# xiexh20/VisTracker

Measured on AMD Instinct MI355X. Metric: frames/sec joint SMPL+object fit, higher is better.
Workload: dtype f32 (decoder GEMMs: 22-bit split-f16 operands x3 MFMA, fp32 accumulate)

## Files before the change

vistracker_amd/csrc/smplh.hip:

```cpp
#include "common.h"
#include <cstring>

#define V_ VT_SMPL_V
#define J_ VT_SMPL_J
#define NB_ VT_SMPL_NB
#define NP_ VT_SMPL_NP
#define VP_ 6912
#define NVT_ 27
#define KQ_ 472
#define NQ_ 480
typedef float f32x4 __attribute__((ext_vector_type(4)));
#define MFMA16(a, b, c) __builtin_amdgcn_mfma_f32_16x16x4f32((a), (b), (c), 0, 0, 0)

#define WS_R 0
#define WS_J (52 * 9)
#define WS_G (WS_J + 52 * 3)
#define WS_A (WS_G + 52 * 12)
#define WS_FRAME (WS_A + 52 * 12)
#define PT_DA 0
#define PT_DTR 624
#define PT_N 627
#define KTOT_ (VP_ * 3)
#define KG_SLAB 24
#define NKS_ (KTOT_ / 16 / KG_SLAB)

#define SCHED_STEPS 32
#define SCHED_WIDTH 10
struct SmplParents { int p[J_]; int nsteps; short sched[SCHED_STEPS][SCHED_WIDTH]; };

#define SP_K 8
struct vt_smplh {
    float *Q_kcv, *Q_t, *W_jv, *W_v64, *J_t, *J_s;
    float *W_sp;
    int nnz;
    SmplParents par;
};

struct RodCtx { float n, ax, ay, az, c, s, qn, w, x, y, z; };

__device__ __forceinline__ void rodrigues_fwd(const float *t, float *R, RodCtx *k)
{
    const float xe = t[0] + 1e-8f, ye = t[1] + 1e-8f, ze = t[2] + 1e-8f;
    const float n = sqrtf(xe * xe + ye * ye + ze * ze);
    const float ax = t[0] / n, ay = t[1] / n, az = t[2] / n;
    const float h = n * 0.5f;
    const float c = cosf(h), s = sinf(h);
    const float q0 = c, q1 = s * ax, q2 = s * ay, q3 = s * az;
    const float qn = sqrtf(q0 * q0 + q1 * q1 + q2 * q2 + q3 * q3);
    const float w = q0 / qn, x = q1 / qn, y = q2 / qn, z = q3 / qn;
    const float w2 = w * w, x2 = x * x, y2 = y * y, z2 = z * z;
    const float wx = w * x, wy = w * y, wz = w * z, xy = x * y, xz = x * z, yz = y * z;
    R[0] = w2 + x2 - y2 - z2; R[1] = 2 * xy - 2 * wz;   R[2] = 2 * wy + 2 * xz;
    R[3] = 2 * wz + 2 * xy;   R[4] = w2 - x2 + y2 - z2; R[5] = 2 * yz - 2 * wx;
    R[6] = 2 * xz - 2 * wy;   R[7] = 2 * wx + 2 * yz;   R[8] = w2 - x2 - y2 + z2;
    if (k) { k->n = n; k->ax = ax; k->ay = ay; k->az = az; k->c = c; k->s = s; k->qn = qn; k->w = w; k->x = x; k->y = y; k->z = z; }
}

__device__ __forceinline__ void rodrigues_bwd(const float *t, const float *dR, float *dt)
{
    float R[9]; RodCtx k; rodrigues_fwd(t, R, &k);
    const float w = k.w, x = k.x, y = k.y, z = k.z;
    const float dw = 2 * w * (dR[0] + dR[4] + dR[8]) + 2 * (-z * dR[1] + y * dR[2] + z * dR[3] - x * dR[5] - y * dR[6] + x * dR[7]);
    const float dx = 2 * x * (dR[0] - dR[4] - dR[8]) + 2 * (y * dR[1] + z * dR[2] + y * dR[3] - w * dR[5] + z * dR[6] + w * dR[7]);
    const float dy = 2 * y * (-dR[0] + dR[4] - dR[8]) + 2 * (x * dR[1] + w * dR[2] + x * dR[3] + z * dR[5] - w * dR[6] + z * dR[7]);
    const float dz = 2 * z * (-dR[0] - dR[4] + dR[8]) + 2 * (-w * dR[1] + x * dR[2] + w * dR[3] + y * dR[5] + x * dR[6] + y * dR[7]);
    const float dot = w * dw + x * dx + y * dy + z * dz;
    const float dq0 = (dw - w * dot) / k.qn, dq1 = (dx - x * dot) / k.qn, dq2 = (dy - y * dot) / k.qn, dq3 = (dz - z * dot) / k.qn;
    const float dh = -k.s * dq0 + k.c * (k.ax * dq1 + k.ay * dq2 + k.az * dq3);
    const float dax = k.s * dq1, day = k.s * dq2, daz = k.s * dq3;
    const float dn = 0.5f * dh - (t[0] * dax + t[1] * day + t[2] * daz) / (k.n * k.n);
    dt[0] = dax / k.n + dn * (t[0] + 1e-8f) / k.n;
    dt[1] = day / k.n + dn * (t[1] + 1e-8f) / k.n;
    dt[2] = daz / k.n + dn * (t[2] + 1e-8f) / k.n;
}

__global__ void rodrigues_fwd_kernel(const float *aa, int n, float *R)
{
    const int i = blockIdx.x * blockDim.x + threadIdx.x;
    if (i >= n) return;
    float t[3] = {aa[3 * i], aa[3 * i + 1], aa[3 * i + 2]}, r[9];
    rodrigues_fwd(t, r, nullptr);
#pragma unroll
    for (int e = 0; e < 9; e++) R[9 * i + e] = r[e];
}

__global__ void rodrigues_bwd_kernel(const float *aa, int n, const float *dR, float *daa)
{
    const int i = blockIdx.x * blockDim.x + threadIdx.x;
    if (i >= n) return;
    float t[3] = {aa[3 * i], aa[3 * i + 1], aa[3 * i + 2]}, g[9], d[3];
#pragma unroll
    for (int e = 0; e < 9; e++) g[e] = dR[9 * i + e];
    rodrigues_bwd(t, g, d);
    daa[3 * i] = d[0]; daa[3 * i + 1] = d[1]; daa[3 * i + 2] = d[2];
}

__global__ __launch_bounds__(64) void smplh_pose_kernel(const float *__restrict__ pose, const float *__restrict__ betas,
                                                        const float *__restrict__ trans, const float *__restrict__ J_t,
                                                        const float *__restrict__ J_s, SmplParents par,
                                                        float *__restrict__ ws, float *__restrict__ jtr, const int *skip)
{
    VT_SKIP_RETURN(skip);
    __shared__ float sR[J_ * 9], sJ[J_ * 3], sG[J_ * 12];
    const int b = blockIdx.x, j = threadIdx.x;
    float *w = ws + (size_t)b * WS_FRAME;
    if (j < J_) {
        float t[3] = {pose[(b * J_ + j) * 3], pose[(b * J_ + j) * 3 + 1], pose[(b * J_ + j) * 3 + 2]}, R[9];
        rodrigues_fwd(t, R, nullptr);
#pragma unroll
        for (int e = 0; e < 9; e++) { sR[j * 9 + e] = R[e]; w[WS_R + j * 9 + e] = R[e]; }
#pragma unroll
        for (int c = 0; c < 3; c++) {
            float a = J_t[j * 3 + c];
#pragma unroll
            for (int l = 0; l < NB_; l++) a += J_s[(j * 3 + c) * NB_ + l] * betas[b * NB_ + l];
            sJ[j * 3 + c] = a; w[WS_J + j * 3 + c] = a;
        }
    }
    __shared__ int sPar[J_];
    if (j < J_) sPar[j] = par.p[j];
    __syncthreads();
    int lvl = 0, maxl = 0;
    if (j < J_) { for (int q = j; q != 0; q = sPar[q]) lvl++; }
    maxl = lvl;
    for (int o = 32; o > 0; o >>= 1) maxl = max(maxl, __shfl_xor(maxl, o, 64));
    maxl = __builtin_amdgcn_readfirstlane(maxl);
    if (j == 0) { for (int r = 0; r < 3; r++) { for (int c = 0; c < 3; c++) sG[r * 4 + c] = sR[r * 3 + c]; sG[r * 4 + 3] = sJ[r]; } }
    __syncthreads();
    for (int l = 1; l <= maxl; l++) {
        if (j < J_ && lvl == l) {
            const int i = j, p = sPar[i];
            const float *Gp = sG + 12 * p, *Ri = sR + 9 * i;
            const float d0 = sJ[3 * i] - sJ[3 * p], d1 = sJ[3 * i + 1] - sJ[3 * p + 1], d2 = sJ[3 * i + 2] - sJ[3 * p + 2];
            float *Gi = sG + 12 * i;
            for (int r = 0; r < 3; r++) {
                const float g0 = Gp[r * 4], g1 = Gp[r * 4 + 1], g2 = Gp[r * 4 + 2];
                Gi[r * 4 + 0] = g0 * Ri[0] + g1 * Ri[3] + g2 * Ri[6];
                Gi[r * 4 + 1] = g0 * Ri[1] + g1 * Ri[4] + g2 * Ri[7];
                Gi[r * 4 + 2] = g0 * Ri[2] + g1 * Ri[5] + g2 * Ri[8];
                Gi[r * 4 + 3] = g0 * d0 + g1 * d1 + g2 * d2 + Gp[r * 4 + 3];
            }
        }
        __syncthreads();
    }
    if (j < J_) {
        const float *G = sG + 12 * j;
#pragma unroll
        for (int r = 0; r < 3; r++) {
            const float gt = G[r * 4 + 3];
            w[WS_G + j * 12 + r * 4 + 0] = G[r * 4]; w[WS_G + j * 12 + r * 4 + 1] = G[r * 4 + 1];
            w[WS_G + j * 12 + r * 4 + 2] = G[r * 4 + 2]; w[WS_G + j * 12 + r * 4 + 3] = gt;
            w[WS_A + j * 12 + r * 4 + 0] = G[r * 4]; w[WS_A + j * 12 + r * 4 + 1] = G[r * 4 + 1]; w[WS_A + j * 12 + r * 4 + 2] = G[r * 4 + 2];
            w[WS_A + j * 12 + r * 4 + 3] = gt - (G[r * 4] * sJ[3 * j] + G[r * 4 + 1] * sJ[3 * j + 1] + G[r * 4 + 2] * sJ[3 * j + 2]);
            if (jtr) jtr[(b * J_ + j) * 3 + r] = gt + trans[3 * b + r];
        }
    }
}

#define FWD_FB 16
#ifndef FWD_PF
#define FWD_PF 6
#endif
#define AXS 516
#define SAS 628
#define FWD_R0 (FWD_FB * AXS > 8 * SAS ? FWD_FB * AXS : 8 * SAS)
__global__ __launch_bounds__(256) void smplh_verts_kernel(const float *__restrict__ Q_kcv, const float *__restrict__ W_jv,
                                                          const float *__restrict__ betas, const float *__restrict__ trans,
                                                          const float *__restrict__ ws, int B,
                                                          float *__restrict__ verts, float *__restrict__ v_posed, const float *__restrict__ W_sp, int nnz, const int *skip)
{
    VT_SKIP_RETURN(skip);
    extern __shared__ __attribute__((aligned(16))) float lds[];
    float *sAx = lds;
    float *sA = lds;
    float *sVp = lds + FWD_R0;
    float *sW = sVp + FWD_FB * 64 * 3;
    float *sTr = sW + (nnz > 0 ? 2 * SP_K * 64 : J_ * 64);
    const int tid = threadIdx.x, wave = tid >> 6, lane = tid & 63, q = lane >> 4, j = lane & 15;
    const int b0 = blockIdx.y * FWD_FB, v = blockIdx.x * 64 + wave * 16 + j;
    for (int k = tid; k < KQ_; k += 256) {
        const int e9 = k % 9;
        const float sub = (k < NP_ && (e9 == 0 || e9 == 4 || e9 == 8)) ? 1.f : 0.f;
        float val[FWD_FB];
#pragma unroll
        for (int f = 0; f < FWD_FB; f++) {
            const int b = min(b0 + f, B - 1);
            if (k < NP_) val[f] = ws[(size_t)b * WS_FRAME + WS_R + 9 + k];
            else if (k < NP_ + NB_) val[f] = betas[b * NB_ + (k - NP_)];
            else val[f] = (k == NP_ + NB_) ? 1.f : 0.f;
        }
#pragma unroll
        for (int f = 0; f < FWD_FB; f++) sAx[f * AXS + k] = val[f] - sub;
    }
    if (nnz > 0) {
        for (int i = tid; i < nnz * 64; i += 256) {
            sW[i] = W_sp[(size_t)(i >> 6) * VP_ + blockIdx.x * 64 + (i & 63)];
            sW[SP_K * 64 + i] = W_sp[(size_t)(SP_K + (i >> 6)) * VP_ + blockIdx.x * 64 + (i & 63)];
        }
    } else
        for (int i = tid; i < J_ * 64; i += 256) sW[i] = W_jv[(i >> 6) * VP_ + blockIdx.x * 64 + (i & 63)];
    if (tid < FWD_FB * 3) { const int f = tid / 3, b = min(b0 + f, B - 1); sTr[tid] = trans[b * 3 + tid % 3]; }
    __syncthreads();

    f32x4 acc[3];
#pragma unroll
    for (int c = 0; c < 3; c++) acc[c] = (f32x4){0.f, 0.f, 0.f, 0.f};
    constexpr int NS = KQ_ / 8;
    float bq[FWD_PF][2][3];
#define FWD_LOADQ(slot_, s_)                                                                     \
    {                                                                                            \
        const float *qk = Q_kcv + (size_t)(8 * (s_) + 2 * q) * 3 * VP_ + v;                      \
        _Pragma("unroll") for (int e = 0; e < 2; e++)                                            \
            _Pragma("unroll") for (int c = 0; c < 3; c++) bq[slot_][e][c] = qk[(size_t)(e * 3 + c) * VP_]; \
    }
#pragma unroll
    for (int s = 0; s < FWD_PF; s++) FWD_LOADQ(s, s)
#pragma unroll
    for (int s = 0; s < NS; s++) {
        const float2 av = *reinterpret_cast<const float2 *>(sAx + j * AXS + 8 * s + 2 * q);
#pragma unroll
        for (int c = 0; c < 3; c++) acc[c] = MFMA16(av.x, bq[s % FWD_PF][0][c], acc[c]);
#pragma unroll
        for (int c = 0; c < 3; c++) acc[c] = MFMA16(av.y, bq[s % FWD_PF][1][c], acc[c]);
        if (s + FWD_PF < NS) FWD_LOADQ(s % FWD_PF, s + FWD_PF)
        __builtin_amdgcn_sched_barrier(0);
    }
#undef FWD_LOADQ
    __syncthreads();
#pragma unroll
    for (int r = 0; r < 4; r++)
#pragma unroll
        for (int c = 0; c < 3; c++) sVp[((4 * q + r) * 64 + wave * 16 + j) * 3 + c] = acc[c][r];
    const int vv = tid & 63, vg = blockIdx.x * 64 + vv;
#pragma unroll 1
    for (int r = 0; r < 4; r++) {
        if ((r & 1) == 0) {
            if (r) __syncthreads();
            for (int i = tid; i < 8 * 624; i += 256) {
                const int sl = i / 624, f = 4 * (sl >> 1) + r + (sl & 1), b = min(b0 + f, B - 1);
                sA[sl * SAS + (i % 624)] = ws[(size_t)b * WS_FRAME + WS_A + (i % 624)];
            }
            __syncthreads();
        }
        const int f = 4 * wave + r, b = b0 + f;
        float T[12];
#pragma unroll
        for (int e = 0; e < 12; e++) T[e] = 0.f;
        const float4 *Af = reinterpret_cast<const float4 *>(sA + (2 * wave + (r & 1)) * SAS);
        if (nnz > 0) {
            for (int k = 0; k < nnz; k++) {
                const int jj = __float_as_int(sW[k * 64 + vv]);
                const float wj = sW[(SP_K + k) * 64 + vv];
                const float4 a0 = Af[jj * 3], a1 = Af[jj * 3 + 1], a2 = Af[jj * 3 + 2];
                T[0] += wj * a0.x; T[1] += wj * a0.y; T[2] += wj * a0.z; T[3] += wj * a0.w;
                T[4] += wj * a1.x; T[5] += wj * a1.y; T[6] += wj * a1.z; T[7] += wj * a1.w;
                T[8] += wj * a2.x; T[9] += wj * a2.y; T[10] += wj * a2.z; T[11] += wj * a2.w;
            }
        } else {
#pragma unroll 4
            for (int jj = 0; jj < J_; jj++) {
                const float wj = sW[jj * 64 + vv];
                const float4 a0 = Af[jj * 3], a1 = Af[jj * 3 + 1], a2 = Af[jj * 3 + 2];
                T[0] += wj * a0.x; T[1] += wj * a0.y; T[2] += wj * a0.z; T[3] += wj * a0.w;
                T[4] += wj * a1.x; T[5] += wj * a1.y; T[6] += wj * a1.z; T[7] += wj * a1.w;
                T[8] += wj * a2.x; T[9] += wj * a2.y; T[10] += wj * a2.z; T[11] += wj * a2.w;
            }
        }
        if (b < B && vg < V_) {
            const float p0 = sVp[(f * 64 + vv) * 3], p1 = sVp[(f * 64 + vv) * 3 + 1], p2 = sVp[(f * 64 + vv) * 3 + 2];
            const size_t o = ((size_t)b * V_ + vg) * 3;
#pragma unroll
            for (int rr = 0; rr < 3; rr++) verts[o + rr] = T[rr * 4] * p0 + T[rr * 4 + 1] * p1 + T[rr * 4 + 2] * p2 + T[rr * 4 + 3] + sTr[f * 3 + rr];
            v_posed[o] = p0; v_posed[o + 1] = p1; v_posed[o + 2] = p2;
        }
    }
}

template <int FB>
__global__ __launch_bounds__(256) void smplh_bwd_tile_kernel(const float *__restrict__ W_v64, const float *__restrict__ ws,
                                                             const float *__restrict__ v_posed, const float *__restrict__ dverts,
                                                             int B, float *__restrict__ part, float *__restrict__ dvp_g, const int *skip)
{
    VT_SKIP_RETURN(skip);
    extern __shared__ __attribute__((aligned(16))) float lds[];
    float *sdT = lds;
    float *sA = sdT + 256 * 13;
    const int tid = threadIdx.x, tile = blockIdx.x, b0 = blockIdx.y * FB, v0 = tile * 256, v = v0 + tid;
    const int wave = tid >> 6, lane = tid & 63, q = lane >> 4, j = lane & 15;
    for (int i = tid; i < FB * 624; i += 256) { const int f = i / 624, b = min(b0 + f, B - 1); sA[i] = ws[(size_t)b * WS_FRAME + WS_A + (i % 624)]; }
    float w1[4][13], w2[64];
#pragma unroll
    for (int mt = 0; mt < 4; mt++)
#pragma unroll
        for (int ks = 0; ks < 13; ks++) w1[mt][ks] = W_v64[(size_t)(v0 + 64 * wave + 16 * mt + j) * 64 + 4 * ks + q];
#pragma unroll
    for (int ks = 0; ks < 64; ks++) w2[ks] = W_v64[(size_t)(v0 + 4 * ks + q) * 64 + wave * 16 + j];
    __syncthreads();
    float dvn[3] = {0.f, 0.f, 0.f}, vpn[3] = {0.f, 0.f, 0.f};
    auto fetch = [&](int b) {
#pragma unroll
        for (int r = 0; r < 3; r++) { dvn[r] = 0.f; vpn[r] = 0.f; }
        if (b < B && v < V_) {
            const size_t o = ((size_t)b * V_ + v) * 3;
            dvn[0] = dverts[o]; dvn[1] = dverts[o + 1]; dvn[2] = dverts[o + 2];
            vpn[0] = v_posed[o]; vpn[1] = v_posed[o + 1]; vpn[2] = v_posed[o + 2];
        }
    };
    fetch(b0);
#pragma unroll 1
    for (int f = 0; f < FB; f++) {
        const int b = b0 + f;
        const float dv[3] = {dvn[0], dvn[1], dvn[2]}, vp[3] = {vpn[0], vpn[1], vpn[2]};
        if (f + 1 < FB) fetch(b + 1);
#pragma unroll
        for (int r = 0; r < 3; r++) {
            sdT[tid * 13 + r * 4 + 0] = dv[r] * vp[0]; sdT[tid * 13 + r * 4 + 1] = dv[r] * vp[1];
            sdT[tid * 13 + r * 4 + 2] = dv[r] * vp[2]; sdT[tid * 13 + r * 4 + 3] = dv[r];
        }
        __syncthreads();
        {
            f32x4 t[4];
#pragma unroll
            for (int mt = 0; mt < 4; mt++) t[mt] = (f32x4){0.f, 0.f, 0.f, 0.f};
#pragma unroll
            for (int ks = 0; ks < 13; ks++) {
                const float bv = j < 12 ? sA[f * 624 + (4 * ks + q) * 12 + j] : 0.f;
#pragma unroll
                for (int mt = 0; mt < 4; mt++) t[mt] = MFMA16(w1[mt][ks], bv, t[mt]);
            }
            const int r4 = (j < 12 ? (j >> 2) : 0) * 4 + 3;
#pragma unroll
            for (int mt = 0; mt < 4; mt++) {
#pragma unroll
                for (int r = 0; r < 4; r++) {
                    const int vl = 64 * wave + 16 * mt + 4 * q + r;
                    float x = t[mt][r] * sdT[vl * 13 + r4];
                    x += __shfl_down(x, 4, 16) + __shfl_down(x, 8, 16);
                    if (j < 3 && b < B) dvp_g[(size_t)b * KTOT_ + (size_t)(v0 + vl) * 3 + j] = x;
                }
            }
        }
        {
            f32x4 acc = (f32x4){0.f, 0.f, 0.f, 0.f}, acc2 = (f32x4){0.f, 0.f, 0.f, 0.f};
#pragma unroll
            for (int ks = 0; ks < 64; ks += 2) {
                const int va = 4 * ks + q, vb = va + 4;
                const float a0 = j < 12 ? sdT[va * 13 + j] : 0.f, a1 = j < 12 ? sdT[vb * 13 + j] : 0.f;
                acc = MFMA16(a0, w2[ks], acc);
                acc2 = MFMA16(a1, w2[ks + 1], acc2);
            }
            acc += acc2;
            if (b < B) {
                float *dst = part + ((size_t)tile * B + b) * PT_N;
                const int jn = wave * 16 + j;
#pragma unroll
                for (int r = 0; r < 4; r++) {
                    const int e = 4 * q + r;
                    if (e < 12) {
                        if (jn < J_) dst[PT_DA + jn * 12 + e] = acc[r];
                        else if (jn == J_ && (e & 3) == 3) dst[PT_DTR + (e >> 2)] = acc[r];
                    }
                }
            }
        }
        __syncthreads();
    }
}

#define BL_M 96
#ifndef BL_NW
#define BL_NW 1
#endif
#define BL_AS 132
__global__ __launch_bounds__(256) void smplh_bwd_blend_kernel(const float *__restrict__ Q_p, const float *__restrict__ dvp_g, int B,
                                                              float *__restrict__ part3, const int *skip)
{
    VT_SKIP_RETURN(skip);
    __shared__ __attribute__((aligned(16))) float sA[BL_M * BL_AS];
    const int tid = threadIdx.x, wave = tid >> 6, lane = tid & 63, q = lane >> 4, j = lane & 15;
    const int ks = blockIdx.x, m0 = blockIdx.z * BL_M, nt0 = blockIdx.y * (4 * BL_NW) + wave * BL_NW;
    f32x4 acc[6][BL_NW];
#pragma unroll
    for (int mt = 0; mt < 6; mt++)
#pragma unroll
        for (int n = 0; n < BL_NW; n++) acc[mt][n] = (f32x4){0.f, 0.f, 0.f, 0.f};
    const float4 *Q4 = reinterpret_cast<const float4 *>(Q_p);
#pragma unroll 1
    for (int c = 0; c < KG_SLAB / 8; c++) {
        __syncthreads();
        for (int i = tid; i < BL_M * 32; i += 256) {
            const int row = i >> 5, c4 = i & 31, b = m0 + row;
            float4 v = make_float4(0.f, 0.f, 0.f, 0.f);
            if (b < B) v = *reinterpret_cast<const float4 *>(dvp_g + (size_t)b * KTOT_ + (size_t)(ks * KG_SLAB + c * 8) * 16 + c4 * 4);
            *reinterpret_cast<float4 *>(sA + row * BL_AS + c4 * 4) = v;
        }
        __syncthreads();
#pragma unroll
        for (int g = 0; g < 8; g++) {
            const size_t kg = (size_t)ks * KG_SLAB + c * 8 + g;
            float bq[BL_NW][4];
#pragma unroll
            for (int n = 0; n < BL_NW; n++) {
                const float4 fq = Q4[(kg * (NQ_ / 16) + min(nt0 + n, NQ_ / 16 - 1)) * 64 + lane];
                bq[n][0] = fq.x; bq[n][1] = fq.y; bq[n][2] = fq.z; bq[n][3] = fq.w;
            }
#pragma unroll
            for (int mt = 0; mt < 6; mt++) {
                const float4 a4 = *reinterpret_cast<const float4 *>(sA + (mt * 16 + j) * BL_AS + g * 16 + q * 4);
                const float av[4] = {a4.x, a4.y, a4.z, a4.w};
#pragma unroll
                for (int s = 0; s < 4; s++)
#pragma unroll
                    for (int n = 0; n < BL_NW; n++) acc[mt][n] = MFMA16(av[s], bq[n][s], acc[mt][n]);
            }
        }
    }
#pragma unroll
    for (int mt = 0; mt < 6; mt++) {
#pragma unroll
        for (int r = 0; r < 4; r++) {
            const int b = m0 + mt * 16 + 4 * q + r;
            if (b < B) {
                float *dst = part3 + ((size_t)ks * B + b) * NQ_;
#pragma unroll
                for (int n = 0; n < BL_NW; n++)
                    if (nt0 + n < NQ_ / 16) dst[(nt0 + n) * 16 + j] = acc[mt][n][r];
            }
        }
    }
}

__global__ __launch_bounds__(256) void smplh_bwd_frame_kernel(const float *__restrict__ pose, const float *__restrict__ J_s,
                                                              SmplParents par, const float *__restrict__ ws,
                                                              const float *__restrict__ part, const float *__restrict__ part3,
                                                              const float *__restrict__ djtr, int B, float *__restrict__ dpose, float *__restrict__ dbetas,
                                                              float *__restrict__ dtrans, const int *skip)
{
    VT_SKIP_RETURN(skip);
    __shared__ float red[PT_N], red3[NQ_];
    __shared__ float sdG[J_ * 12], sdJ[J_ * 3], sdR[J_ * 9];
    __shared__ float sG[J_ * 12], sRm[J_ * 9], sJr[J_ * 3];
    const int b = blockIdx.x, tid = threadIdx.x;
    const float *w = ws + (size_t)b * WS_FRAME;
    for (int i = tid; i < J_ * 12; i += 256) sG[i] = w[WS_G + i];
    for (int i = tid; i < J_ * 9; i += 256) sRm[i] = w[WS_R + i];
    for (int i = tid; i < J_ * 3; i += 256) sJr[i] = w[WS_J + i];
    for (int i = tid; i < PT_N; i += 256) {
        float s = 0.f;
#pragma unroll 9
        for (int t = 0; t < NVT_; t++) s += part[((size_t)t * B + b) * PT_N + i];
        red[i] = s;
    }
    for (int i = tid; i < NQ_; i += 256) {
        float s = 0.f;
#pragma unroll 9
        for (int t = 0; t < NKS_; t++) s += part3[((size_t)t * B + b) * NQ_ + i];
        red3[i] = s;
    }
    __syncthreads();
    if (tid < J_) {
        const int j = tid;
        const float *G = sG + 12 * j; const float *Jr = sJr;
        float dj[3] = {0.f, 0.f, 0.f};
#pragma unroll
        for (int r = 0; r < 3; r++) {
            const float dat = red[PT_DA + 12 * j + r * 4 + 3];
#pragma unroll
            for (int c = 0; c < 3; c++) { sdG[12 * j + r * 4 + c] = red[PT_DA + 12 * j + r * 4 + c] - dat * Jr[3 * j + c]; dj[c] -= G[r * 4 + c] * dat; }
            sdG[12 * j + r * 4 + 3] = dat + (djtr ? djtr[(b * J_ + j) * 3 + r] : 0.f);
        }
        sdJ[3 * j] = dj[0]; sdJ[3 * j + 1] = dj[1]; sdJ[3 * j + 2] = dj[2];
#pragma unroll
        for (int e = 0; e < 9; e++) sdR[9 * j + e] = 0.f;
    }
    __syncthreads();
    const int jloc = tid / 24, el = tid - 24 * jloc;
    const int nsteps = par.nsteps > 0 ? par.nsteps : J_ - 1;
    for (int step = 0; step < nsteps; step++) {
        const int j = par.nsteps > 0 ? (jloc < SCHED_WIDTH ? (int)par.sched[step][jloc < SCHED_WIDTH ? jloc : 0] : -1) : (jloc == 0 ? J_ - 1 - step : -1);
        if (j >= 1) {
            const int p = par.p[j];
            const float *Gp = sG + 12 * p, *Rj = sRm + 9 * j, *dGj = sdG + 12 * j;
            float upd = 0.f; float *dst = nullptr; float upd2 = 0.f; float *dst2 = nullptr;
            if (el < 12) {
                const int r = el >> 2, c = el & 3;
                dst = sdG + 12 * p + el;
                if (c < 3) upd = dGj[r * 4] * Rj[3 * c] + dGj[r * 4 + 1] * Rj[3 * c + 1] + dGj[r * 4 + 2] * Rj[3 * c + 2] + dGj[r * 4 + 3] * (sJr[3 * j + c] - sJr[3 * p + c]);
                else upd = dGj[r * 4 + 3];
            } else if (el < 21) {
                const int e = el - 12, r = e / 3, c = e - 3 * r;
                dst = sdR + 9 * j + e;
                upd = Gp[r] * dGj[c] + Gp[4 + r] * dGj[4 + c] + Gp[8 + r] * dGj[8 + c];
            } else {
                const int c = el - 21;
                upd = Gp[c] * dGj[3] + Gp[4 + c] * dGj[7] + Gp[8 + c] * dGj[11];
                dst = sdJ + 3 * j + c; dst2 = sdJ + 3 * p + c; upd2 = -upd;
            }
            if (dst) *dst += upd;
            if (dst2) *dst2 += upd2;
        }
        __syncthreads();
    }
    if (tid < 3) { for (int c = 0; c < 3; c++) sdR[3 * tid + c] += sdG[tid * 4 + c]; sdJ[tid] += sdG[tid * 4 + 3]; }
    __syncthreads();
    if (tid < J_) {
        const int j = tid;
        float g[9], t[3] = {pose[(b * J_ + j) * 3], pose[(b * J_ + j) * 3 + 1], pose[(b * J_ + j) * 3 + 2]}, d[3];
#pragma unroll
        for (int e = 0; e < 9; e++) g[e] = sdR[9 * j + e] + (j >= 1 ? red3[(j - 1) * 9 + e] : 0.f);
        rodrigues_bwd(t, g, d);
        dpose[(b * J_ + j) * 3] = d[0]; dpose[(b * J_ + j) * 3 + 1] = d[1]; dpose[(b * J_ + j) * 3 + 2] = d[2];
    } else if (tid >= 64 && tid < 64 + NB_) {
        const int l = tid - 64;
        float s = red3[NP_ + l];
        for (int i = 0; i < J_ * 3; i++) s += J_s[i * NB_ + l] * sdJ[i];
        dbetas[b * NB_ + l] = s;
    } else if (tid >= 128 && tid < 131) {
        const int c = tid - 128;
        float s = red[PT_DTR + c];
        if (djtr) for (int j = 0; j < J_; j++) s += djtr[(b * J_ + j) * 3 + c];
        dtrans[b * 3 + c] = s;
    }
}

extern "C" int vt_smplh_create(vt_smplh **out, const float *v_template, const float *shapedirs, const float *posedirs,
                               const float *J_regressor, const float *weights, const int *parents, void *stream)
{
    VT_REQUIRE(out && v_template && shapedirs && posedirs && J_regressor && weights && parents, "vt_smplh_create: null argument");
    hipStream_t st = vt_stream(stream);
    vt_smplh *h = new vt_smplh();
    for (int j = 0; j < J_; j++) h->par.p[j] = (j == 0) ? 0 : parents[j];
    for (int j = 1; j < J_; j++) VT_REQUIRE(h->par.p[j] >= 0 && h->par.p[j] < j, "vt_smplh_create: parents[%d]=%d must be in [0,%d)", j, parents[j], j);
    {
        int lvl[J_], rank[J_], maxl = 0;
        lvl[0] = 0; rank[0] = 0;
        for (int j = 1; j < J_; j++) { lvl[j] = lvl[h->par.p[j]] + 1; maxl = std::max(maxl, lvl[j]); rank[j] = 0; for (int k = j + 1; k < J_; k++) rank[j] += (h->par.p[k] == h->par.p[j]); }
        int n = 0; bool ok = true;
        for (int t = 0; t < SCHED_STEPS; t++) for (int i = 0; i < SCHED_WIDTH; i++) h->par.sched[t][i] = -1;
        for (int l = maxl; l >= 1 && ok; l--)
            for (int r = 0; r < J_ && ok; r++) {
                int cnt = 0;
                for (int j = J_ - 1; j >= 1; j--) if (lvl[j] == l && rank[j] == r) { if (n >= SCHED_STEPS || cnt >= SCHED_WIDTH) { ok = false; break; } h->par.sched[n][cnt++] = (short)j; }
                if (cnt) n++;
            }
        h->par.nsteps = ok ? n : 0;
    }
    float *Q_kcv = new float[(size_t)KQ_ * 3 * VP_](), *Q_t = new float[(size_t)VP_ * 3 * NQ_](), *W_jv = new float[(size_t)J_ * VP_](),
          *J_t = new float[J_ * 3], *J_s = new float[J_ * 3 * NB_];
    for (int v = 0; v < V_; v++) for (int c = 0; c < 3; c++) {
        for (int k = 0; k < NP_ + NB_ + 1; k++) {
            const float val = k < NP_ ? posedirs[((size_t)v * 3 + c) * NP_ + k]
                            : (k < NP_ + NB_ ? shapedirs[((size_t)v * 3 + c) * NB_ + (k - NP_)] : v_template[v * 3 + c]);
            Q_kcv[(size_t)(k * 3 + c) * VP_ + v] = val;
            {
                const size_t kr = (size_t)v * 3 + c, g = kr >> 4, qq = (kr & 15) >> 2, ss = kr & 3;
                Q_t[((g * (NQ_ / 16) + (k >> 4)) * 64 + qq * 16 + (k & 15)) * 4 + ss] = val;
            }
        }
    }
    float *W_v64 = new float[(size_t)VP_ * 64]();
    for (int v = 0; v < V_; v++) { for (int j = 0; j < J_; j++) { W_jv[(size_t)j * VP_ + v] = weights[(size_t)v * J_ + j]; W_v64[(size_t)v * 64 + j] = weights[(size_t)v * J_ + j]; } W_v64[(size_t)v * 64 + J_] = 1.0f; }
    float *W_sp = new float[(size_t)2 * SP_K * VP_]();
    int nnz = 0;
    for (int v = 0; v < V_; v++) {
        int k = 0;
        for (int j = 0; j < J_; j++) {
            const float w = weights[(size_t)v * J_ + j];
            if (w == 0.0f) continue;
            if (k < SP_K) { const int jj = j; memcpy(&W_sp[(size_t)k * VP_ + v], &jj, 4); W_sp[(size_t)(SP_K + k) * VP_ + v] = w; }
            k++;
        }
        nnz = k > nnz ? k : nnz;
    }
    h->nnz = nnz <= SP_K ? (nnz > 0 ? nnz : 1) : 0;
    for (int j = 0; j < J_; j++) for (int c = 0; c < 3; c++) {
        double a = 0; double sb[NB_] = {0};
        for (int v = 0; v < V_; v++) {
            const double r = J_regressor[(size_t)j * V_ + v];
            if (r == 0.0) continue;
            a += r * v_template[v * 3 + c];
            for (int l = 0; l < NB_; l++) sb[l] += r * shapedirs[((size_t)v * 3 + c) * NB_ + l];
        }
        J_t[j * 3 + c] = (float)a;
        for (int l = 0; l < NB_; l++) J_s[(j * 3 + c) * NB_ + l] = (float)sb[l];
    }
    int rc = VT_OK;
    if ((rc = vt_upload(&h->Q_kcv, Q_kcv, (size_t)KQ_ * 3 * VP_, st)) || (rc = vt_upload(&h->Q_t, Q_t, (size_t)VP_ * 3 * NQ_, st)) ||
        (rc = vt_upload(&h->W_jv, W_jv, (size_t)J_ * VP_, st)) || (rc = vt_upload(&h->W_v64, W_v64, (size_t)VP_ * 64, st)) ||
        (rc = vt_upload(&h->J_t, J_t, (size_t)J_ * 3, st)) || (rc = vt_upload(&h->J_s, J_s, (size_t)J_ * 3 * NB_, st)) ||
        (rc = vt_upload(&h->W_sp, W_sp, (size_t)2 * SP_K * VP_, st))) {
        return rc;
    }
    VT_HIP(hipStreamSynchronize(st));
    delete[] Q_kcv; delete[] Q_t; delete[] W_jv; delete[] W_v64; delete[] J_t; delete[] J_s; delete[] W_sp;
    *out = h;
    return VT_OK;
}

extern "C" void vt_smplh_destroy(vt_smplh *h)
{
    if (!h) return;
    hipFree(h->Q_kcv); hipFree(h->Q_t); hipFree(h->W_jv); hipFree(h->W_v64); hipFree(h->J_t); hipFree(h->J_s); hipFree(h->W_sp);
    delete h;
}

extern "C" long vt_smplh_workspace_floats(int B) { return (long)B * WS_FRAME; }
extern "C" long vt_smplh_bwd_scratch_floats(int B) { return (long)NVT_ * B * PT_N + (long)B * KTOT_ + (long)NKS_ * B * NQ_; }

#define BWD_FB 6

extern "C" int vt_smplh_forward(const vt_smplh *h, const float *pose, const float *betas, const float *trans, int B,
                                float *verts, float *jtr, float *v_posed, float *ws, void *stream)
{
    VT_REQUIRE(h && pose && betas && trans && verts && v_posed && ws && B > 0, "vt_smplh_forward: null argument or B <= 0");
    hipStream_t st = vt_stream(stream); const int *skip = vt_skip_flag_of(st);
    hipLaunchKernelGGL(smplh_pose_kernel, dim3(B), dim3(64), 0, st, pose, betas, trans, h->J_t, h->J_s, h->par, ws, jtr, skip);
    VT_LAUNCH_CHECK();
    const size_t lds_f = sizeof(float) * (FWD_R0 + FWD_FB * 64 * 3 + (h->nnz > 0 ? 2 * SP_K * 64 : J_ * 64) + FWD_FB * 3);
    VT_LDS_LIMIT(smplh_verts_kernel, sizeof(float) * (FWD_R0 + FWD_FB * 64 * 3 + J_ * 64 + FWD_FB * 3));
    hipLaunchKernelGGL(smplh_verts_kernel, dim3(VP_ / 64, (B + FWD_FB - 1) / FWD_FB), dim3(256), lds_f, st, h->Q_kcv, h->W_jv, betas, trans, ws, B,
                       verts, v_posed, h->W_sp, h->nnz, skip);
    VT_LAUNCH_CHECK();
    return VT_OK;
}

extern "C" int vt_smplh_backward(const vt_smplh *h, const float *pose, const float *betas, int B, const float *dverts,
                                 const float *djtr, const float *v_posed, const float *ws, float *scratch,
                                 float *dpose, float *dbetas, float *dtrans, void *stream)
{
    (void)betas;
    VT_REQUIRE(h && pose && dverts && v_posed && ws && scratch && dpose && dbetas && dtrans && B > 0, "vt_smplh_backward: null argument or B <= 0");
    hipStream_t st = vt_stream(stream); const int *skip = vt_skip_flag_of(st);
    const size_t lds = sizeof(float) * (256 * 13 + BWD_FB * 624);
    float *dvp_g = scratch + (size_t)NVT_ * B * PT_N, *part3 = dvp_g + (size_t)B * KTOT_;
    VT_LDS_LIMIT(smplh_bwd_tile_kernel<BWD_FB>, lds);
    hipLaunchKernelGGL(smplh_bwd_tile_kernel<BWD_FB>, dim3(NVT_, (B + BWD_FB - 1) / BWD_FB), dim3(256), lds, st, h->W_v64, ws, v_posed, dverts, B, scratch, dvp_g, skip);
    VT_LAUNCH_CHECK();
    hipLaunchKernelGGL(smplh_bwd_blend_kernel, dim3(NKS_, (NQ_ / 16 + 4 * BL_NW - 1) / (4 * BL_NW), (B + BL_M - 1) / BL_M), dim3(256), 0, st, h->Q_t, dvp_g, B, part3, skip);
    VT_LAUNCH_CHECK();
    hipLaunchKernelGGL(smplh_bwd_frame_kernel, dim3(B), dim3(256), 0, st, pose, h->J_s, h->par, ws, scratch, part3, djtr, B, dpose, dbetas, dtrans, skip);
    VT_LAUNCH_CHECK();
    return VT_OK;
}

extern "C" int vt_rodrigues_forward(const float *aa, int n, float *R, void *stream)
{
    VT_REQUIRE(aa && R && n > 0, "vt_rodrigues_forward: bad argument");
    hipLaunchKernelGGL(rodrigues_fwd_kernel, dim3((n + 255) / 256), dim3(256), 0, vt_stream(stream), aa, n, R);
    VT_LAUNCH_CHECK();
    return VT_OK;
}

extern "C" int vt_rodrigues_backward(const float *aa, int n, const float *dR, float *daa, void *stream)
{
    VT_REQUIRE(aa && dR && daa && n > 0, "vt_rodrigues_backward: bad argument");
    hipLaunchKernelGGL(rodrigues_bwd_kernel, dim3((n + 255) / 256), dim3(256), 0, vt_stream(stream), aa, n, dR, daa);
    VT_LAUNCH_CHECK();
    return VT_OK;
}
```

Baseline: 151.3.

## Batch frames into MFMA rows in SMPL-H backward tile kernel and shrink blend LDS

The backward tile kernel drops its per-frame loop. It stacks four frames' 12 dT rows into a 48-row MFMA M dimension, so W_v64 columns are reused across frames in one pass. The first GEMM now computes all three pose components per frame at once, replacing the shuffle reduction. The second GEMM streams w2 in 128-vertex chunks to cut register pressure, paired with a waves_per_eu(4) hint. The blend kernel stages 4 K-groups per LDS fill instead of 8, which reduces shared memory and may raise occupancy at the cost of more barriers.

```diff
diff --git a/vistracker_amd/csrc/smplh.hip b/vistracker_amd/csrc/smplh.hip
--- a/vistracker_amd/csrc/smplh.hip
+++ b/vistracker_amd/csrc/smplh.hip
@@ -276,94 +276,111 @@
     }
 }
 
-template <int FB>
-__global__ __launch_bounds__(256) void smplh_bwd_tile_kernel(const float *__restrict__ W_v64, const float *__restrict__ ws,
+#define BWD_FB 4
+#define BWD_CH 128
+#define BWD_DS 132
+#define BWD_LDS (BWD_FB * 12 * BWD_DS)
+__global__ __launch_bounds__(256) __attribute__((amdgpu_waves_per_eu(4))) void smplh_bwd_tile_kernel(const float *__restrict__ W_v64, const float *__restrict__ ws,
                                                              const float *__restrict__ v_posed, const float *__restrict__ dverts,
                                                              int B, float *__restrict__ part, float *__restrict__ dvp_g, const int *skip)
 {
     VT_SKIP_RETURN(skip);
     extern __shared__ __attribute__((aligned(16))) float lds[];
+    float *sA = lds;
+    float *sDv = sA + BWD_FB * 624;
     float *sdT = lds;
-    float *sA = sdT + 256 * 13;
-    const int tid = threadIdx.x, tile = blockIdx.x, b0 = blockIdx.y * FB, v0 = tile * 256, v = v0 + tid;
+    const int tid = threadIdx.x, tile = blockIdx.x, b0 = blockIdx.y * BWD_FB, v0 = tile * 256, v = v0 + tid;
     const int wave = tid >> 6, lane = tid & 63, q = lane >> 4, j = lane & 15;
-    for (int i = tid; i < FB * 624; i += 256) { const int f = i / 624, b = min(b0 + f, B - 1); sA[i] = ws[(size_t)b * WS_FRAME + WS_A + (i % 624)]; }
-    float w1[4][13], w2[64];
+    for (int i = tid; i < BWD_FB * 624; i += 256) { const int f = i / 624, b = min(b0 + f, B - 1); sA[i] = ws[(size_t)b * WS_FRAME + WS_A + (i % 624)]; }
+    float dv[BWD_FB][3], vp[BWD_FB][3];
+#pragma unroll
+    for (int f = 0; f < BWD_FB; f++) {
+        const int b = b0 + f;
+        const bool ok = b < B && v < V_;
+        const size_t o = ((size_t)(ok ? b : 0) * V_ + (ok ? v : 0)) * 3;
+#pragma unroll
+        for (int r = 0; r < 3; r++) { dv[f][r] = ok ? dverts[o + r] : 0.f; vp[f][r] = ok ? v_posed[o + r] : 0.f; }
+#pragma unroll
+        for (int r = 0; r < 3; r++) sDv[(f * 256 + tid) * 3 + r] = dv[f][r];
+    }
+    float w1[4][13];
 #pragma unroll
     for (int mt = 0; mt < 4; mt++)
 #pragma unroll
         for (int ks = 0; ks < 13; ks++) w1[mt][ks] = W_v64[(size_t)(v0 + 64 * wave + 16 * mt + j) * 64 + 4 * ks + q];
-#pragma unroll
-    for (int ks = 0; ks < 64; ks++) w2[ks] = W_v64[(size_t)(v0 + 4 * ks + q) * 64 + wave * 16 + j];
-    __syncthreads();
-    float dvn[3] = {0.f, 0.f, 0.f}, vpn[3] = {0.f, 0.f, 0.f};
-    auto fetch = [&](int b) {
-#pragma unroll
-        for (int r = 0; r < 3; r++) { dvn[r] = 0.f; vpn[r] = 0.f; }
-        if (b < B && v < V_) {
-            const size_t o = ((size_t)b * V_ + v) * 3;
-            dvn[0] = dverts[o]; dvn[1] = dverts[o + 1]; dvn[2] = dverts[o + 2];
-            vpn[0] = v_posed[o]; vpn[1] = v_posed[o + 1]; vpn[2] = v_posed[o + 2];
-        }
-    };
-    fetch(b0);
+    __syncthreads();
+    {
+        const int f = j < 12 ? j / 3 : 0, c = j < 12 ? j - 3 * f : 0, b = b0 + f;
+        const float *sAf = sA + f * 624 + q * 12 + c;
+#pragma unroll
+        for (int h = 0; h < 2; h++) {
+            f32x4 t[3][2];
+#pragma unroll
+            for (int r = 0; r < 3; r++) { t[r][0] = (f32x4){0.f, 0.f, 0.f, 0.f}; t[r][1] = (f32x4){0.f, 0.f, 0.f, 0.f}; }
+#pragma unroll
+            for (int ks = 0; ks < 13; ks++) {
+#pragma unroll
+                for (int r = 0; r < 3; r++) {
+                    const float bv = j < 12 ? sAf[ks * 48 + 4 * r] : 0.f;
+                    t[r][0] = MFMA16(w1[2 * h][ks], bv, t[r][0]);
+                    t[r][1] = MFMA16(w1[2 * h + 1][ks], bv, t[r][1]);
+                }
+            }
+#pragma unroll
+            for (int m2 = 0; m2 < 2; m2++) {
+#pragma unroll
+                for (int rr = 0; rr < 4; rr++) {
+                    const int vl = 64 * wave + 16 * (2 * h + m2) + 4 * q + rr;
+                    const float *d = sDv + (f * 256 + vl) * 3;
+                    const float x0 = t[0][m2][rr] * d[0], x1 = t[1][m2][rr] * d[1], x2 = t[2][m2][rr] * d[2];
+                    if (j < 12 && b < B) dvp_g[(size_t)b * KTOT_ + (size_t)(v0 + vl) * 3 + c] = x0 + (x1 + x2);
+                }
+            }
+        }
+    }
+    f32x4 acc[3], acc2[3];
+#pragma unroll
+    for (int mt = 0; mt < 3; mt++) { acc[mt] = (f32x4){0.f, 0.f, 0.f, 0.f}; acc2[mt] = (f32x4){0.f, 0.f, 0.f, 0.f}; }
 #pragma unroll 1
-    for (int f = 0; f < FB; f++) {
-        const int b = b0 + f;
-        const float dv[3] = {dvn[0], dvn[1], dvn[2]}, vp[3] = {vpn[0], vpn[1], vpn[2]};
-        if (f + 1 < FB) fetch(b + 1);
-#pragma unroll
-        for (int r = 0; r < 3; r++) {
-            sdT[tid * 13 + r * 4 + 0] = dv[r] * vp[0]; sdT[tid * 13 + r * 4 + 1] = dv[r] * vp[1];
-            sdT[tid * 13 + r * 4 + 2] = dv[r] * vp[2]; sdT[tid * 13 + r * 4 + 3] = dv[r];
-        }
+    for (int ch = 0; ch < 256 / BWD_CH; ch++) {
+        float w2[BWD_CH / 4];
+#pragma unroll
+        for (int kk = 0; kk < BWD_CH / 4; kk++) w2[kk] = W_v64[(size_t)(v0 + BWD_CH * ch + 4 * kk + q) * 64 + wave * 16 + j];
         __syncthreads();
-        {
-            f32x4 t[4];
-#pragma unroll
-            for (int mt = 0; mt < 4; mt++) t[mt] = (f32x4){0.f, 0.f, 0.f, 0.f};
-#pragma unroll
-            for (int ks = 0; ks < 13; ks++) {
-                const float bv = j < 12 ? sA[f * 624 + (4 * ks + q) * 12 + j] : 0.f;
-#pragma unroll
-                for (int mt = 0; mt < 4; mt++) t[mt] = MFMA16(w1[mt][ks], bv, t[mt]);
-            }
-            const int r4 = (j < 12 ? (j >> 2) : 0) * 4 + 3;
-#pragma unroll
-            for (int mt = 0; mt < 4; mt++) {
-#pragma unroll
-                for (int r = 0; r < 4; r++) {
-                    const int vl = 64 * wave + 16 * mt + 4 * q + r;
-                    float x = t[mt][r] * sdT[vl * 13 + r4];
-                    x += __shfl_down(x, 4, 16) + __shfl_down(x, 8, 16);
-                    if (j < 3 && b < B) dvp_g[(size_t)b * KTOT_ + (size_t)(v0 + vl) * 3 + j] = x;
+        if (tid / BWD_CH == ch) {
+            const int vl = tid % BWD_CH;
+#pragma unroll
+            for (int f = 0; f < BWD_FB; f++)
+#pragma unroll
+                for (int r = 0; r < 3; r++) {
+                    float *row = sdT + (12 * f + 4 * r) * BWD_DS + vl;
+                    row[0] = dv[f][r] * vp[f][0]; row[BWD_DS] = dv[f][r] * vp[f][1]; row[2 * BWD_DS] = dv[f][r] * vp[f][2]; row[3 * BWD_DS] = dv[f][r];
                 }
-            }
-        }
-        {
-            f32x4 acc = (f32x4){0.f, 0.f, 0.f, 0.f}, acc2 = (f32x4){0.f, 0.f, 0.f, 0.f};
-#pragma unroll
-            for (int ks = 0; ks < 64; ks += 2) {
-                const int va = 4 * ks + q, vb = va + 4;
-                const float a0 = j < 12 ? sdT[va * 13 + j] : 0.f, a1 = j < 12 ? sdT[vb * 13 + j] : 0.f;
-                acc = MFMA16(a0, w2[ks], acc);
-                acc2 = MFMA16(a1, w2[ks + 1], acc2);
-            }
-            acc += acc2;
+        }
+        __syncthreads();
+#pragma unroll
+        for (int kk = 0; kk < BWD_CH / 4; kk += 2) {
+#pragma unroll
+            for (int mt = 0; mt < 3; mt++) {
+                const float *a = sdT + (16 * mt + j) * BWD_DS + 4 * kk + q;
+                acc[mt] = MFMA16(a[0], w2[kk], acc[mt]);
+                acc2[mt] = MFMA16(a[4], w2[kk + 1], acc2[mt]);
+            }
+        }
+    }
+    const int jn = wave * 16 + j;
+#pragma unroll
+    for (int mt = 0; mt < 3; mt++) {
+        acc[mt] += acc2[mt];
+#pragma unroll
+        for (int rr = 0; rr < 4; rr++) {
+            const int m = 16 * mt + 4 * q + rr, f = m / 12, e = m - 12 * f, b = b0 + f;
             if (b < B) {
                 float *dst = part + ((size_t)tile * B + b) * PT_N;
-                const int jn = wave * 16 + j;
-#pragma unroll
-                for (int r = 0; r < 4; r++) {
-                    const int e = 4 * q + r;
-                    if (e < 12) {
-                        if (jn < J_) dst[PT_DA + jn * 12 + e] = acc[r];
-                        else if (jn == J_ && (e & 3) == 3) dst[PT_DTR + (e >> 2)] = acc[r];
-                    }
-                }
-            }
-        }
-        __syncthreads();
+                if (jn < J_) dst[PT_DA + jn * 12 + e] = acc[mt][rr];
+                else if (jn == J_ && (e & 3) == 3) dst[PT_DTR + (e >> 2)] = acc[mt][rr];
+            }
+        }
     }
 }
 
@@ -371,12 +388,12 @@
 #ifndef BL_NW
 #define BL_NW 1
 #endif
-#define BL_AS 132
+#define BL_KG 4
+#define BL_AS (16 * BL_KG + 4)
 __global__ __launch_bounds__(256) void smplh_bwd_blend_kernel(const float *__restrict__ Q_p, const float *__restrict__ dvp_g, int B,
                                                               float *__restrict__ part3, const int *skip)
 {
     VT_SKIP_RETURN(skip);
-    __shared__ __attribute__((aligned(16))) float sA[BL_M * BL_AS];
     const int tid = threadIdx.x, wave = tid >> 6, lane = tid & 63, q = lane >> 4, j = lane & 15;
     const int ks = blockIdx.x, m0 = blockIdx.z * BL_M, nt0 = blockIdx.y * (4 * BL_NW) + wave * BL_NW;
     f32x4 acc[6][BL_NW];
@@ -385,19 +402,20 @@
 #pragma unroll
         for (int n = 0; n < BL_NW; n++) acc[mt][n] = (f32x4){0.f, 0.f, 0.f, 0.f};
     const float4 *Q4 = reinterpret_cast<const float4 *>(Q_p);
+    __shared__ __attribute__((aligned(16))) float sA[BL_M * BL_AS];
 #pragma unroll 1
-    for (int c = 0; c < KG_SLAB / 8; c++) {
+    for (int c = 0; c < KG_SLAB / BL_KG; c++) {
         __syncthreads();
-        for (int i = tid; i < BL_M * 32; i += 256) {
-            const int row = i >> 5, c4 = i & 31, b = m0 + row;
+        for (int i = tid; i < BL_M * 4 * BL_KG; i += 256) {
+            const int row = i / (4 * BL_KG), c4 = i % (4 * BL_KG), b = m0 + row;
             float4 v = make_float4(0.f, 0.f, 0.f, 0.f);
-            if (b < B) v = *reinterpret_cast<const float4 *>(dvp_g + (size_t)b * KTOT_ + (size_t)(ks * KG_SLAB + c * 8) * 16 + c4 * 4);
+            if (b < B) v = *reinterpret_cast<const float4 *>(dvp_g + (size_t)b * KTOT_ + (size_t)(ks * KG_SLAB + c * BL_KG) * 16 + c4 * 4);
             *reinterpret_cast<float4 *>(sA + row * BL_AS + c4 * 4) = v;
         }
         __syncthreads();
 #pragma unroll
-        for (int g = 0; g < 8; g++) {
-            const size_t kg = (size_t)ks * KG_SLAB + c * 8 + g;
+        for (int g = 0; g < BL_KG; g++) {
+            const size_t kg = (size_t)ks * KG_SLAB + c * BL_KG + g;
             float bq[BL_NW][4];
 #pragma unroll
             for (int n = 0; n < BL_NW; n++) {
@@ -607,8 +625,6 @@
 extern "C" long vt_smplh_workspace_floats(int B) { return (long)B * WS_FRAME; }
 extern "C" long vt_smplh_bwd_scratch_floats(int B) { return (long)NVT_ * B * PT_N + (long)B * KTOT_ + (long)NKS_ * B * NQ_; }
 
-#define BWD_FB 6
-
 extern "C" int vt_smplh_forward(const vt_smplh *h, const float *pose, const float *betas, const float *trans, int B,
                                 float *verts, float *jtr, float *v_posed, float *ws, void *stream)
 {
@@ -631,10 +647,9 @@
     (void)betas;
     VT_REQUIRE(h && pose && dverts && v_posed && ws && scratch && dpose && dbetas && dtrans && B > 0, "vt_smplh_backward: null argument or B <= 0");
     hipStream_t st = vt_stream(stream); const int *skip = vt_skip_flag_of(st);
-    const size_t lds = sizeof(float) * (256 * 13 + BWD_FB * 624);
+    const size_t lds = sizeof(float) * BWD_LDS;
     float *dvp_g = scratch + (size_t)NVT_ * B * PT_N, *part3 = dvp_g + (size_t)B * KTOT_;
-    VT_LDS_LIMIT(smplh_bwd_tile_kernel<BWD_FB>, lds);
-    hipLaunchKernelGGL(smplh_bwd_tile_kernel<BWD_FB>, dim3(NVT_, (B + BWD_FB - 1) / BWD_FB), dim3(256), lds, st, h->W_v64, ws, v_posed, dverts, B, scratch, dvp_g, skip);
+    hipLaunchKernelGGL(smplh_bwd_tile_kernel, dim3(NVT_, (B + BWD_FB - 1) / BWD_FB), dim3(256), lds, st, h->W_v64, ws, v_posed, dverts, B, scratch, dvp_g, skip);
     VT_LAUNCH_CHECK();
     hipLaunchKernelGGL(smplh_bwd_blend_kernel, dim3(NKS_, (NQ_ / 16 + 4 * BL_NW - 1) / (4 * BL_NW), (B + BL_M - 1) / BL_M), dim3(256), 0, st, h->Q_t, dvp_g, B, part3, skip);
     VT_LAUNCH_CHECK();
```

After: 153.5 (median of 6 runs). +1.5%, better.
